# Aakash1312/Fluid-Simulation

Measured on AMD Instinct MI355X. Metric: simulated substeps/sec, higher is better.
Workload: dtype f64

## Files before the change

fluid-simulation_amd/csrc/common.h:

```cpp
#pragma once
#include <hip/hip_runtime.h>
#include <stdint.h>

namespace fl {

constexpr uint8_t F_SOLID = 1;
constexpr uint8_t F_FLUID = 2;
constexpr int F_CNT_SHIFT = 2;

struct Grid {
    int N;
    int lo;
    int hi;
    int nx, ny, nz;
    int ox, oy, oz;
    __host__ __device__ inline size_t idx(int ix, int iy, int iz) const
    {
        return ((size_t)ix * ny + (size_t)iy) * nz + (size_t)iz;
    }
    __host__ __device__ inline size_t cells() const { return (size_t)nx * ny * nz; }
    __host__ __device__ inline long sx() const { return (long)ny * nz; }
    __host__ __device__ inline int cx0() const { return lo + ox; }
    __host__ __device__ inline int cy0() const { return lo + oy; }
    __host__ __device__ inline int cz0() const { return lo + oz; }
// ... 115 lines not shown
    T r = 0;
    if (threadIdx.x == 0) {
#pragma unroll
        for (int i = 0; i < NW; ++i) r += sm[i];
    }
    return r;
}
template <int NW>
__device__ __forceinline__ double block_sum_array(const double* __restrict__ a, int n, double* sm)
{
    double v = 0;
    for (int i = threadIdx.x; i < n; i += NW * 64) v += a[i];
    v = wave_sum(v);
    const int lane = threadIdx.x & 63, w = threadIdx.x >> 6;
    __syncthreads();
    if (lane == 0) sm[w] = v;
    __syncthreads();
    if (threadIdx.x == 0) {
        double r = 0;
#pragma unroll
        for (int i = 0; i < NW; ++i) r += sm[i];
        sm[NW] = r;
    }
    __syncthreads();
    return sm[NW];
}

__device__ __forceinline__ int xcd_remap(int b, int nb)
{
    const int q = nb >> 3, r = nb & 7, xcd = b & 7;
    return (xcd < r ? xcd * (q + 1) : r * (q + 1) + (xcd - r) * q) + (b >> 3);
}

__device__ __forceinline__ void block_sum3(const double* __restrict__ a, int na, const double* __restrict__ b, int nb,
                                           const double* __restrict__ c, int nc, double* sm, double& ra, double& rb, double& rc)
{
    double va = 0, vb = 0, vc = 0;
    for (int i = threadIdx.x; i < na; i += 256) va += a[i];
    for (int i = threadIdx.x; i < nb; i += 256) vb += b[i];
    for (int i = threadIdx.x; i < nc; i += 256) vc += c[i];
    va = wave_sum(va); vb = wave_sum(vb); vc = wave_sum(vc);
    const int lane = threadIdx.x & 63, w = threadIdx.x >> 6;
    if (lane == 0) { sm[w] = va; sm[4 + w] = vb; sm[8 + w] = vc; }
    __syncthreads();
    ra = ((sm[0] + sm[1]) + sm[2]) + sm[3];
    rb = ((sm[4] + sm[5]) + sm[6]) + sm[7];
    rc = ((sm[8] + sm[9]) + sm[10]) + sm[11];
}

struct Particles {
    double *px, *py, *pz, *vx, *vy, *vz;
    uint32_t* pid;
    __host__ __device__ inline Particles shifted(long o) const
    {
        Particles q = *this;
        q.px += o; q.py += o; q.pz += o; q.vx += o; q.vy += o; q.vz += o; q.pid += o;
        return q;
    }
};
constexpr uint32_t PID_DEAD = 0xFFFFFFFFu;

void launch_bin_count(hipStream_t st, Grid g, long n, Particles p, int* key, int* slot, int* cell_count, int* part, StepState* ss);
void launch_bin_scatter(hipStream_t st, long n, const int* key, const int* slot, const int* cell_start, const uint32_t* pid, int* order,
                         uint32_t* spid);
void launch_bin_rank(hipStream_t st, long n_pos, long pos0, const int* key, const int* cell_start, const int* order, const uint32_t* spid,
                     int* order2);
void launch_reorder(hipStream_t st, long n, const int* order, Particles src, Particles dst, double* w = nullptr, long wstride = 0);
void launch_weights(hipStream_t st, long n, Particles p, double* w, long stride);
void launch_axpby_box(hipStream_t st, Grid g, Box box, double a, const double* x, double b, const double* y, double* out, const PcgState* gate = nullptr);
long p2g_max_items(Box box);
size_t p2g_part_doubles(Box box);
constexpr int P2G_PILED = 256;
void launch_p2g(hipStream_t st, Grid g, Box box, Particles p, const double* pw, long wstride, const int* cell_start, const uint8_t* flags,
                double* part, int* items, float* container, double* u, double* v, double* w, double* ub, double* vb, double* wb, int2* crowd_list = nullptr,
                Particles park = Particles{});
void launch_p2g_tiles(hipStream_t st, Grid g, Box box, Particles p, const double* pw, long wstride, const int* cell_start, const uint8_t* flags,
                      float* container, double* u, double* v, double* w, double* ub, double* vb, double* wb);
void launch_g2p_tiled(hipStream_t st, Grid g, Box pb, Particles p, const int* cell_start, const double* dcx, const double* dcy, const double* dcz,
                      const double* pcx, const double* pcy, const double* pcz, double blend, StepState* ss);
void launch_g2p(hipStream_t st, Grid g, long n, Particles p, const double* dcx, const double* dcy, const double* dcz, const double* pcx,
// ... 186 lines not shown
```

fluid-simulation_amd/csrc/kernels_mg.hip:

```cpp
#include "common.h"
#include <cstdlib>
#include <cstring>

namespace fl {

constexpr double MG_W1 = 0.5617, MG_W2 = 1.3895;

template <typename T>
__device__ __forceinline__ void mg_load_coef(T* sd, T* si, const MgCoef<T>& cf)
{
    if (threadIdx.x == 0) {
#pragma unroll
        for (int i = 0; i < 7; ++i) {
            sd[i] = cf.diag[i];
            si[i] = cf.inv[i];
        }
    }
    __syncthreads();
}

__device__ __forceinline__ bool mg_cell(const MLevel& m, long t, int& i, int& j, int& k)
{
    const unsigned n = (unsigned)m.dx * (unsigned)m.dy * (unsigned)m.dz;
    if (t >= (long)n) return false;
// ... 114 lines not shown
    z = r - y * RZ;
}
__device__ __forceinline__ bool in_level(const MLevel& m, int i, int j, int k)
{
    return (unsigned)i < (unsigned)m.dx && (unsigned)j < (unsigned)m.dy && (unsigned)k < (unsigned)m.dz;
}

__device__ __forceinline__ int clampi(int v, int hi) { return min(max(v, 0), hi); }

template <typename T, int TX, int TY, int TZ, bool RESTRICT>
struct DownTile {
    static constexpr int H = RESTRICT ? 3 : 2;
    static constexpr int AX = TX + 2 * H, AY = TY + 2 * H, AZ = TZ + 2 * H;
    static constexpr int BX = AX - 2, BY = AY - 2, BZ = AZ - 2;
    static constexpr int CX = BX - 2, CY = BY - 2, CZ = BZ - 2;
    static constexpr int nA = AX * AY * AZ, nB = BX * BY * BZ, nR = RESTRICT ? CX * CY * CZ : 4;
    static constexpr int oA = 0, oB = (oA + nA * (int)sizeof(T) + 15) / 16 * 16, oR = (oB + nB * (int)sizeof(T) + 15) / 16 * 16,
                         oC = (oR + nR * (int)sizeof(T) + 15) / 16 * 16, bytes = (oC + nA + 15) / 16 * 16;
};
template <typename T, int TX, int TY, int TZ>
struct UpTile {
    static constexpr int AX = TX + 4, AY = TY + 4, AZ = TZ + 4;
    static constexpr int BX = TX + 2, BY = TY + 2, BZ = TZ + 2;
    static constexpr int EX = TX / 2 + 4, EY = TY / 2 + 4, EZ = TZ / 2 + 4;
    static constexpr int nA = AX * AY * AZ, nB = BX * BY * BZ, nE = EX * EY * EZ;
    static constexpr int oA = 0, oB = (oA + nA * (int)sizeof(T) + 15) / 16 * 16, oE = (oB + nB * (int)sizeof(T) + 15) / 16 * 16,
                         oC = (oE + nE * (int)sizeof(T) + 15) / 16 * 16, bytes = (oC + nA + 15) / 16 * 16;
};

template <typename T, typename F, int TX, int TY, int TZ, bool RESTRICT, typename IO, int NG, typename RhsFn, typename CoreFn>
__device__ __forceinline__ void mg_down_body_fn(const MLevel& m, const uint8_t* __restrict__ cnt, T* __restrict__ u,
                                                T* __restrict__ r, const MLevel& mc, const uint8_t* __restrict__ cnt_c, T* __restrict__ fc,
                                                const MgCoef<T>* cf, T off, int tile, int gx, int gy, bool live, int col, char* lds, T* sd, T* si,
                                                int grp, RhsFn rhs, CoreFn core)
{
    typedef DownTile<T, TX, TY, TZ, RESTRICT> D;
    constexpr int H = D::H, AX = D::AX, AY = D::AY, AZ = D::AZ, BX = D::BX, BY = D::BY, BZ = D::BZ, CX = D::CX, CY = D::CY, CZ = D::CZ;
    constexpr int PA = (AX + NG - 1) / NG, PB = (BX + NG - 1) / NG;
    constexpr int NHC = NG * (256 / (CY * CZ)), XC = (CX + NHC - 1) / NHC;
    static_assert(AY * AZ <= 256 && NHC >= 1 && TX % 2 == 0 && TY % 2 == 0 && TZ % 2 == 0, "tile shape");
    T* sA = (T*)(lds + D::oA);
    T* sB = (T*)(lds + D::oB);
    T* sR = (T*)(lds + D::oR);
    uint8_t* sC = (uint8_t*)(lds + D::oC);
    const int tbx = tile % gx, tby = (tile / gx) % gy, tbz = tile / (gx * gy);
    const int i0 = tbz * TX, j0 = tby * TY, k0 = tbx * TZ;
    const T w1 = (T)MG_W1, w2 = (T)MG_W2;
    const long sx = m.sx;
    const int ya = col / AZ, za = col - ya * AZ;
    const bool actA = col < AY * AZ;
    const bool okA = actA && (unsigned)(j0 - H + ya) < (unsigned)m.dy && (unsigned)(k0 - H + za) < (unsigned)m.dz;
    const size_t qa = m.at(0, clampi(j0 - H + ya, m.dy - 1), clampi(k0 - H + za, m.dz - 1));
    const int xa0 = grp * PA;
    int ca[PA];
    T fa[PA];
#pragma unroll
    for (int p = 0; p < PA; ++p) {
        const int x = xa0 + p, i = i0 - H + x;
        const size_t q = qa + (size_t)((long)clampi(i, m.dx - 1) * sx);
        const int c = cnt[q];
        fa[p] = (T)rhs(q);
        ca[p] = (okA && x < AX && (unsigned)i < (unsigned)m.dx) ? c : 0;
    }
    const int yb = col / BZ, zb = col - yb * BZ;
    const bool actB = col < BY * BZ;
    const size_t qb = m.at(0, clampi(j0 - H + 1 + yb, m.dy - 1), clampi(k0 - H + 1 + zb, m.dz - 1));
    const int xb0 = grp * PB;
    T fb[PB];
#pragma unroll
    for (int p = 0; p < PB; ++p) fb[p] = (T)rhs(qb + (size_t)((long)clampi(i0 - H + 1 + xb0 + p, m.dx - 1) * sx));
    const int hc = grp * (256 / (CY * CZ)) + col / (CY * CZ), cc = col % (CY * CZ);
    const int yc = cc / CZ, zc = cc - yc * CZ;
    const bool actC = col / (CY * CZ) < 256 / (CY * CZ);
    const int xc0 = hc * XC;
    const size_t qc = m.at(0, clampi(j0 - H + 2 + yc, m.dy - 1), clampi(k0 - H + 2 + zc, m.dz - 1));
    T fr[XC];
#pragma unroll
    for (int x = 0; x < XC; ++x) fr[x] = (T)rhs(qc + (size_t)((long)clampi(i0 - H + 2 + xc0 + x, m.dx - 1) * sx));
    if (cf) mg_load_coef(sd, si, *cf);
    if (actA) {
#pragma unroll
        for (int p = 0; p < PA; ++p) {
            const int x = xa0 + p;
            if (x < AX) {
                sC[x * AY * AZ + col] = (uint8_t)ca[p];
                sA[x * AY * AZ + col] = w1 * si[ca[p]] * fa[p];
            }
        }
    }
    __syncthreads();
    if (actB && xb0 < BX) {
        const int a0 = (yb + 1) * AZ + zb + 1 + xb0 * AY * AZ;
        T cm = sA[a0], c0 = sA[a0 + AY * AZ];
        const bool in_yz = live && (unsigned)(yb - (H - 1)) < (unsigned)TY && (unsigned)(zb - (H - 1)) < (unsigned)TZ;
#pragma unroll
        for (int p = 0; p < PB; ++p) {
            const int x = xb0 + p;
            if (x < BX) {
                const int a = a0 + (p + 1) * AY * AZ;
                const T cp = sA[a + AY * AZ];
                const int n = sC[a];
                const T nb = cm + cp + sA[a - AZ] + sA[a + AZ] + sA[a - 1] + sA[a + 1];
                const T v = c0 + w2 * si[n] * (fb[p] - (sd[n] * c0 + off * nb));
                sB[(x * BY + yb) * BZ + zb] = v;
                if (n && in_yz && x >= H - 1 && x < H - 1 + TX) IO::st(u + qb + (size_t)((long)(i0 - H + 1 + x) * sx), v);
                cm = c0;
                c0 = cp;
            }
        }
    }
    __syncthreads();
    T rk[XC];
#pragma unroll
    for (int x = 0; x < XC; ++x) rk[x] = 0;
    if (actC && xc0 < CX) {
        const int b0 = ((xc0 + 1) * BY + yc + 1) * BZ + zc + 1;
        T cm = sB[b0 - BY * BZ], c0 = sB[b0];
#pragma unroll
        for (int x = 0; x < XC; ++x) {
            if (xc0 + x < CX) {
                const int b = b0 + x * BY * BZ;
                const T cp = sB[b + BY * BZ];
                const int n = sC[((xc0 + x + 2) * AY + yc + 2) * AZ + zc + 2];
// ... 31 lines not shown
            }
        }
    }
    if (RESTRICT) {
        __syncthreads();
        constexpr int QX = TX / 2, QY = TY / 2, QZ = TZ / 2;
        for (int t = grp * 256 + col; t < QX * QY * QZ; t += 256 * NG) {
            int X, Y, Z;
            region_cell<QY, QZ>(t, X, Y, Z);
            const int I = i0 / 2 + X, J = j0 / 2 + Y, K = k0 / 2 + Z;
            if (!live || !in_level(mc, I, J, K)) continue;
            const size_t C = mc.at(I, J, K);
            if (!cnt_c[C]) continue;
            auto w = [](int a) { return (a == 0 || a == 3) ? (T)0.25 : (T)0.75; };
            const T* p = sR + ((2 * X) * CY + 2 * Y) * CZ + 2 * Z;
            T acc = 0;
#pragma unroll
            for (int a = 0; a < 4; ++a) {
#pragma unroll
                for (int b = 0; b < 4; ++b) {
                    const T* q = p + (a * CY + b) * CZ;
                    acc += w(a) * w(b) * ((T)0.25 * (q[0] + q[3]) + (T)0.75 * (q[1] + q[2]));
                }
            }
            IO::st(fc + C, acc * (T)0.125);
        }
    }
}

template <typename T, typename F, int TX, int TY, int TZ, bool RESTRICT, typename IO, int NG = 1>
__device__ __forceinline__ void mg_down_body(const MLevel& m, const uint8_t* __restrict__ cnt, const F* __restrict__ f, T* __restrict__ u,
                                             T* __restrict__ r, const MLevel& mc, const uint8_t* __restrict__ cnt_c, T* __restrict__ fc,
                                             const MgCoef<T>* cf, T off, int tile, int gx, int gy, bool live, int col, char* lds, T* sd, T* si,
                                             int grp = 0)
{
    mg_down_body_fn<T, F, TX, TY, TZ, RESTRICT, IO, NG>(m, cnt, u, r, mc, cnt_c, fc, cf, off, tile, gx, gy, live, col, lds, sd, si, grp,
                                                        [&](size_t q) { return IO::ld(f + q); }, [](size_t) {});
}

template <typename T, typename F, int TX, int TY, int TZ, bool RESTRICT, int NG = 1>
__global__ __launch_bounds__(256 * NG) void k_mg_down(MLevel m, const uint8_t* __restrict__ cnt, const F* __restrict__ f, T* __restrict__ u,
                                                      T* __restrict__ r, MLevel mc, const uint8_t* __restrict__ cnt_c, T* __restrict__ fc,
                                                      MgCoef<T> cf, const PcgState* ps, int gx, int gy, const int* __restrict__ tlist)
{
    __shared__ __attribute__((aligned(16))) char lds[DownTile<T, TX, TY, TZ, RESTRICT>::bytes];
    __shared__ T sd[8], si[8];
    if (ps && ps->done) return;
    const int tile = tlist ? tlist[xcd_remap(blockIdx.x, gridDim.x)] : xcd_remap(blockIdx.x, gridDim.x);
    mg_down_body<T, F, TX, TY, TZ, RESTRICT, IoPlain, NG>(m, cnt, f, u, r, mc, cnt_c, fc, &cf, cf.off, tile, gx, gy, true, NG > 1 ? (int)(threadIdx.x & 255) : (int)threadIdx.x,
                                                          lds, sd, si, NG > 1 ? __builtin_amdgcn_readfirstlane(threadIdx.x >> 8) : 0);
}

template <typename T, typename F, typename O, int TX, int TY, int TZ, typename IO, int NG = 1>
__device__ __forceinline__ void mg_up_body(const MLevel& m, const uint8_t* __restrict__ cnt, const F* __restrict__ f, const T* __restrict__ u,
                                           O* __restrict__ out, const MLevel& mc, const T* __restrict__ ec, const MgCoef<T>* cf, T off,
                                           double* __restrict__ part_dot, int tile, int gx, int gy, T wc, const uint8_t* __restrict__ own, bool live,
                                           int col, char* lds, T* sd, T* si, double* red, int grp = 0, bool pconst = false)
{
    typedef UpTile<T, TX, TY, TZ> D;
    constexpr int AX = D::AX, AY = D::AY, AZ = D::AZ, BX = D::BX, BY = D::BY, BZ = D::BZ, EX = D::EX, EY = D::EY, EZ = D::EZ;
    constexpr int NE = (EX * EY * EZ + 256 * NG - 1) / (256 * NG);
    constexpr int PA = (AX + NG - 1) / NG, PB = (BX + NG - 1) / NG;
    constexpr int NHT = NG * (256 / (TY * TZ)), XT = (TX + NHT - 1) / NHT;
    static_assert(AY * AZ <= 256 && 256 % (TY * TZ) == 0 && TX % 2 == 0 && TY % 2 == 0 && TZ % 2 == 0, "tile shape");
    T* sA = (T*)(lds + D::oA);
    T* sB = (T*)(lds + D::oB);
    T* sE = (T*)(lds + D::oE);
    uint8_t* sC = (uint8_t*)(lds + D::oC);
    const int tbx = tile % gx, tby = (tile / gx) % gy, tbz = tile / (gx * gy);
    const int i0 = tbz * TX, j0 = tby * TY, k0 = tbx * TZ;
    const int I0 = i0 / 2 - 2, J0 = j0 / 2 - 2, K0 = k0 / 2 - 2;
    const long sx = m.sx;
    const int tid = grp * 256 + col;
    T ee[NE];
#pragma unroll
    for (int it = 0; it < NE; ++it) {
        int x, y, z;
        region_cell<EY, EZ>(tid + 256 * NG * it, x, y, z);
        const int I = I0 + x, J = J0 + y, K = K0 + z;
        const bool ok = I >= -1 && I <= mc.dx && J >= -1 && J <= mc.dy && K >= -1 && K <= mc.dz;
        const T v = IO::ld(ec + mc.at(min(max(I, -1), mc.dx), min(max(J, -1), mc.dy), min(max(K, -1), mc.dz)));
        ee[it] = ok ? v : (T)0;
    }
    const int ya = col / AZ, za = col - ya * AZ;
    const bool actA = col < AY * AZ;
    const bool okA = actA && (unsigned)(j0 - 2 + ya) < (unsigned)m.dy && (unsigned)(k0 - 2 + za) < (unsigned)m.dz;
    const size_t qa = m.at(0, clampi(j0 - 2 + ya, m.dy - 1), clampi(k0 - 2 + za, m.dz - 1));
    const int xa0 = grp * PA;
    int ca[PA];
    T ua[PA];
#pragma unroll
    for (int p = 0; p < PA; ++p) {
        const int x = xa0 + p, i = i0 - 2 + x;
        const size_t q = qa + (size_t)((long)clampi(i, m.dx - 1) * sx);
        const int c = cnt[q];
        ua[p] = IO::ld(u + q);
        ca[p] = (okA && (NG == 1 || x < AX) && (unsigned)i < (unsigned)m.dx) ? c : 0;
    }
    const int yb = col / BZ, zb = col - yb * BZ;
    const bool actB = col < BY * BZ;
    const size_t qb = m.at(0, clampi(j0 - 1 + yb, m.dy - 1), clampi(k0 - 1 + zb, m.dz - 1));
    const int xb0 = grp * PB;
    T fb[PB];
#pragma unroll
    for (int p = 0; p < PB; ++p) fb[p] = (T)IO::ld(f + qb + (size_t)((long)clampi(i0 - 1 + xb0 + p, m.dx - 1) * sx));
    const int hl = col / (TY * TZ), ct = col - hl * (TY * TZ);
    const int ht = NG == 1 ? hl : grp * (256 / (TY * TZ)) + hl;
    const int yt = ct / TZ, zt = ct - yt * TZ;
    const int xt0 = ht * XT;
    const size_t qt = m.at(0, clampi(j0 + yt, m.dy - 1), clampi(k0 + zt, m.dz - 1));
    F ft[XT];
#pragma unroll
    for (int x = 0; x < XT; ++x) ft[x] = IO::ld(f + qt + (size_t)((long)clampi(i0 + xt0 + x, m.dx - 1) * sx));
    if (cf) mg_load_coef(sd, si, *cf);
#pragma unroll
    for (int it = 0; it < NE; ++it) {
        const int t = tid + 256 * NG * it;
        if (t < EX * EY * EZ) sE[t] = ee[it];
    }
    __syncthreads();
    if (actA) {
        const int eb = ((ya >> 1) + 1) * EZ + (za >> 1) + 1;
        const int sy = (ya & 1) ? EZ : -EZ, sz = (za & 1) ? 1 : -1;
        const T a = (T)0.75, b = (T)0.25;
        T pl[EX];
#pragma unroll
        for (int I = 0; I < EX; ++I) {
            const T* p = sE + I * EY * EZ + eb;
            pl[I] = pconst ? p[0] : a * a * p[0] + a * b * (p[sy] + p[sz]) + b * b * p[sy + sz];
        }
#pragma unroll
        for (int p = 0; p < PA; ++p) {
            const int x = xa0 + p;
            if (NG == 1 || x < AX) {
                const int I = (x >> 1) + 1, In = (x & 1) ? I + 1 : I - 1;
                T pI = pl[0], pN = pl[0];
                if constexpr (NG == 1) {
                    pI = pl[(p >> 1) + 1], pN = pl[(p & 1) ? (p >> 1) + 2 : (p >> 1)];
                } else {
#pragma unroll
                    for (int e = 1; e < EX; ++e) { pI = e == I ? pl[e] : pI; pN = e == In ? pl[e] : pN; }
                }
                const T pe = pconst ? pI : a * pI + b * pN;
                sC[x * AY * AZ + col] = (uint8_t)ca[p];
                sA[x * AY * AZ + col] = ca[p] ? ua[p] + wc * pe : (T)0;
            }
        }
    }
    __syncthreads();
    if (actB && (NG == 1 || xb0 < BX)) {
        const int a0 = (yb + 1) * AZ + zb + 1 + xb0 * AY * AZ;
        T cm = sA[a0], c0 = sA[a0 + AY * AZ];
#pragma unroll
// ... 18 lines not shown
#pragma unroll
        for (int x = 0; x < XT; ++x) {
            if (NG == 1 || xt0 + x < TX) {
                const int b = b0 + x * BY * BZ;
                const T cp = sB[b + BY * BZ];
                const int n = sC[((xt0 + x + 2) * AY + yt + 2) * AZ + zt + 2];
                const T nb = cm + cp + sB[b - BZ] + sB[b + BZ] + sB[b - 1] + sB[b + 1];
                const T o = c0 + (T)MG_W1 * si[n] * ((T)ft[x] - (sd[n] * c0 + off * nb));
                if (n && live) {
                    const size_t qo = qt + (size_t)((long)(i0 + xt0 + x) * sx);
                    IO::st(out + qo, (O)o);
                    if (!own || (own[qo] && !(own[qo] & 0x80))) acc += (double)ft[x] * (double)o;
                }
                cm = c0;
                c0 = cp;
            }
        }
    }
    if (NG == 1 && part_dot) {
        acc = block_sum<double, 4>(acc, red);
        if (threadIdx.x == 0) part_dot[blockIdx.x] = acc;
    }
}

template <typename T, typename F, typename O, int TX, int TY, int TZ>
__global__ __launch_bounds__(256, 5) void k_mg_up(MLevel m, const uint8_t* __restrict__ cnt, const F* __restrict__ f, const T* __restrict__ u,
                                                                      O* __restrict__ out, MLevel mc, const T* __restrict__ ec, MgCoef<T> cf,
                                                                      double* __restrict__ part_dot, const PcgState* ps, int gx, int gy, T wc,
                                                                      const int* __restrict__ tlist, const uint8_t* __restrict__ own, int pconst)
{
    __shared__ __attribute__((aligned(16))) char lds[UpTile<T, TX, TY, TZ>::bytes];
    __shared__ T sd[8], si[8];
    __shared__ double red[4];
    if (ps && ps->done) return;
    const int tile = tlist ? tlist[xcd_remap(blockIdx.x, gridDim.x)] : xcd_remap(blockIdx.x, gridDim.x);
    mg_up_body<T, F, O, TX, TY, TZ, IoPlain, 1>(m, cnt, f, u, out, mc, ec, &cf, cf.off, part_dot, tile, gx, gy, wc, own, true, (int)threadIdx.x, lds, sd, si, red, 0,
                                                pconst != 0);
}

template <typename T>
__global__ __launch_bounds__(256) void k_mg_restrict(MLevel mf, const T* __restrict__ rf, MLevel mc, const uint8_t* __restrict__ cnt_c,
                                                     T* __restrict__ fc, const PcgState* ps)
{
    if (ps && ps->done) return;
    d_restrict<T>(mf, rf, mc, cnt_c, fc, (long)blockIdx.x * 256 + threadIdx.x);
}

constexpr int MG_TAIL_Q0 = 4;
template <typename T>
struct MgTail {
    int nl;
    MLevel mg[MG_TAIL_MAX];
    const uint8_t* cnt[MG_TAIL_MAX];
    const T* f0;
    T* u0;
    MLevel ml[MG_TAIL_MAX];
    int o_u[MG_TAIL_MAX], o_v[MG_TAIL_MAX], o_f[MG_TAIL_MAX], o_c[MG_TAIL_MAX];
    int lds_bytes;
    T off[MG_TAIL_MAX];
    int sweeps;
    double wc;
};

struct TailCell {
    int c;
    int n;
    int up;
    int down;
    int bits;
};
// ... 367 lines not shown
```

fluid-simulation_amd/csrc/kernels_pcg.hip:

```cpp
#include "common.h"
#include "stencil_vec.h"

namespace fl {

constexpr int TX = 4, TY = 8, TZ = 32;
constexpr int PY = TY + 2, PZ = TZ + 2;
constexpr int SQ_MAX_BLOCKS = 1024;
constexpr int XR_MAX_BLOCKS = 512;

LBox make_lbox(const Box& b)
{
    LBox L;
    L.x0 = b.x0; L.y0 = b.y0; L.z0 = b.z0;
    L.nx = b.nx(); L.ny = b.ny(); L.nz = b.nz();
    L.Lx = (L.nx + TX - 1) / TX * TX + 2;
    L.Ly = (L.ny + TY - 1) / TY * TY + 2;
    const int tiled = (L.nz + TZ - 1) / TZ * TZ + 1;
    const int need = LBOX_K0 + L.nz + 1 > tiled ? LBOX_K0 + L.nz + 1 : tiled;
    L.Lz = (need + 15) / 16 * 16;
    return L;
}
size_t lbox_max_cells(int N)
{
    Box b{0, 0, 0, N - 1, N - 1, N - 1};
// ... 73 lines not shown
    for (long t0 = (long)blockIdx.x * 256 + threadIdx.x; t0 < n; t0 += 4 * stride) {
        uint8_t c4[4];
#pragma unroll
        for (int q = 0; q < 4; ++q) { const long t = t0 + q * stride; c4[q] = cnt[t < n ? t : n - 1]; }
#pragma unroll
        for (int q = 0; q < 4; ++q) {
            const long t = t0 + q * stride;
            if (t >= n) break;
            const uint8_t c = c4[q];
            T rv = 0, xv = 0;
            if (c && !(c & 0x80)) {
                const int k = (int)(t % L.Lz), j = (int)((t / L.Lz) % L.Ly), i = (int)(t / ((long)L.Lz * L.Ly));
                const size_t gc = g.idx(L.x0 + i - 1, L.y0 + j - 1, L.z0 + k - LBOX_K0);
                const size_t gx = (size_t)g.sx(), gy = (size_t)g.nz;
                const T bv = (T)b[gc];
                auto G = [&](size_t q2) { return guess2 ? (T)(ca * guess[q2] + cb * guess2[q2]) : (T)guess[q2]; };
                const uint8_t n0 = cnt[t - sx], n1 = cnt[t + sx], n2 = cnt[t - sy], n3 = cnt[t + sy], n4 = cnt[t - 1], n5 = cnt[t + 1];
                const T g0 = G(gc - gx), g1 = G(gc + gx), g2 = G(gc - gy), g3 = G(gc + gy), g4 = G(gc - 1), g5 = G(gc + 1);
                xv = G(gc);
                const T nb = (n0 ? g0 : (T)0) + (n1 ? g1 : (T)0) + (n2 ? g2 : (T)0) + (n3 ? g3 : (T)0) + (n4 ? g4 : (T)0) + (n5 ? g5 : (T)0);
                rv = bv - (sdiag[c] * xv + cf.off * nb);
                abb += (double)bv * (double)bv;
                arr += (double)rv * (double)rv;
            }
            x[t] = xv;
            r[t] = rv;
        }
    }
    abb = block_sum<double, 4>(abb, red);
    arr = block_sum<double, 4>(arr, red);
    if (threadIdx.x == 0) { part_bb[blockIdx.x] = abb; part_rr0[blockIdx.x] = arr; }
}

template <typename T>
__device__ __forceinline__ bool pcg_head(const double* __restrict__ part_rr, const double* __restrict__ part_rz_new,
                                         const double* __restrict__ part_rz_old, int n_prev, int n_rz, PcgState* ps, int first, double tol,
                                         double* red, T& beta)
{
    const int tid = threadIdx.x;
    beta = 0;
    if (first) {
        double bb, rr0, d2;
        block_sum3(part_rr, n_prev, part_rz_old, first == 2 ? n_prev : 0, part_rr, 0, red, bb, rr0, d2);
        if (first != 2) rr0 = bb;
        const bool go = bb > 0 && !(rr0 < tol * tol * bb);
        if (blockIdx.x == 0 && tid == 0) {
            ps->bb = bb;
            ps->thr = tol * tol * bb;
            ps->rr = rr0;
            if (!go) ps->done = 1;
        }
        return go;
    }
    double rr, rzn, rzo;
    block_sum3(part_rr, n_prev, part_rz_new, n_rz, part_rz_old, n_rz, red, rr, rzn, rzo);
    if (rr < ps->thr) {
        if (blockIdx.x == 0 && tid == 0) { ps->rr = rr; ps->done = 1; }
        return false;
    }
    beta = (T)(rzn / rzo);
    if (blockIdx.x == 0 && tid == 0) { ps->rr = rr; ps->iters += 1; }
    return true;
}

template <typename T, bool DIST, bool AZ = false, typename ZT = T>
__global__ __launch_bounds__(256) void k_pcg_sq_l(LBox L, const uint8_t* __restrict__ cnt, const ZT* __restrict__ r,
                                                  const T* __restrict__ s_in, T* __restrict__ s_out, T* __restrict__ q, Coef<T> cf,
                                                  const double* __restrict__ part_rr, const double* __restrict__ part_rz_new,
                                                  const double* __restrict__ part_rz_old, double* __restrict__ part_pq, int n_prev,
                                                  PcgState* ps, int first, double tol, int n_rz, int zmode, int sparse,
                                                  const int* __restrict__ tlist, int nlist)
{
    __shared__ T sT[TX * PY * PZ];
    __shared__ double red[16];
    __shared__ int s_done;
    __shared__ T sdiag[8], sinv[8];
    const int tid = threadIdx.x;
    load_coef(sdiag, sinv, cf);
    if (tid == 0) s_done = ps->done;

    const int nty = (L.ny + TY - 1) / TY, ntz = (L.nz + TZ - 1) / TZ;
    const int ntiles = ((L.nx + TX - 1) / TX) * nty * ntz;
    const long sx = (long)L.Ly * L.Lz;
    const int ly = tid >> 5, kz = tid & 31;

    int lidx = xcd_remap(blockIdx.x, gridDim.x);
    int tile = tlist ? (lidx < nlist ? tlist[lidx] : ntiles) : lidx;
    auto entry = [&](int li) { return tlist ? (li < nlist ? tlist[li < nlist ? li : 0] : ntiles) : li; };
    int nxt = entry(lidx + (int)gridDim.x);
    uint8_t fc[TX + 2], fy = 0, fz = 0;
    ZT rv[TX + 2], ry = 0, rz = 0;
    T sv[TX + 2], sy = 0, sz = 0;
    long c0 = 0;
    auto issue = [&](int tl, bool counts, bool values) {
        const int tz = tl % ntz, ty = (tl / ntz) % nty, tx = tl / (ntz * nty);
        const int i0 = 1 + tx * TX, j0 = 1 + ty * TY, k0 = LBOX_K0 + tz * TZ;
        c0 = ((long)(i0 - 1) * L.Ly + (j0 + ly)) * L.Lz + k0 + kz;
#pragma unroll
        for (int m = 0; m < TX + 2; ++m) {
            if (counts) fc[m] = cnt[c0 + m * sx];
            if (values) {
                rv[m] = r[c0 + m * sx];
                sv[m] = first ? (T)0 : s_in[c0 + m * sx];
            }
        }
        {
            const int pl = tid >> 6, side = (tid >> 5) & 1;
            const long cy = ((long)(i0 + pl) * L.Ly + (side ? j0 + TY : j0 - 1)) * L.Lz + k0 + kz;
            if (counts) fy = cnt[cy];
            if (values) { ry = r[cy]; sy = first ? (T)0 : s_in[cy]; }
        }
        if (tid < 64) {
            const int lx = tid >> 4, l2 = (tid >> 1) & 7, side = tid & 1;
            const long cz = ((long)(i0 + lx) * L.Ly + (j0 + l2)) * L.Lz + (side ? k0 + TZ : k0 - 1);
            if (counts) fz = cnt[cz];
            if (values) { rz = r[cz]; sz = first ? (T)0 : s_in[cz]; }
        }
    };
    if (!sparse && tile < ntiles) issue(tile, true, true);

    T beta = 0;
    __syncthreads();
    if (s_done) return;
    if (!AZ && !pcg_head<T>(part_rr, part_rz_new, part_rz_old, n_prev, n_rz, ps, first, tol, red, beta)) return;

    double acc = 0;
    while (tile < ntiles) {
        if (sparse) {
            issue(tile, true, false);
            int any = 0;
#pragma unroll
            for (int m = 1; m <= TX; ++m) any |= fc[m];
            if (!__syncthreads_or(any)) {
                tile = nxt;
                lidx += gridDim.x;
                nxt = entry(lidx + (int)gridDim.x);
                continue;
            }
            issue(tile, false, true);
        }
        T val[TX + 2];
#pragma unroll
        for (int m = 0; m < TX + 2; ++m) val[m] = fc[m] ? (zmode ? (T)rv[m] : (T)rv[m] * sinv[DIST ? fc[m] & 7 : fc[m]]) + beta * sv[m] : (T)0;
#pragma unroll
        for (int lx = 0; lx < TX; ++lx) sT[(lx * PY + ly + 1) * PZ + kz + 1] = val[lx + 1];
        {
            const int pl = tid >> 6, side = (tid >> 5) & 1;
            sT[(pl * PY + (side ? TY + 1 : 0)) * PZ + kz + 1] = fy ? (zmode ? (T)ry : (T)ry * sinv[DIST ? fy & 7 : fy]) + beta * sy : (T)0;
        }
        if (tid < 64) {
            const int lx = tid >> 4, l2 = (tid >> 1) & 7, side = tid & 1;
            sT[(lx * PY + l2 + 1) * PZ + (side ? TZ + 1 : 0)] = fz ? (zmode ? (T)rz : (T)rz * sinv[DIST ? fz & 7 : fz]) + beta * sz : (T)0;
        }
        __syncthreads();
        const long cc = c0;
        uint8_t fcc[TX];
        T nbv[TX], cen[TX];
// ... 131 lines not shown
        }
        ((V2*)s)[i] = sv; ((V2*)q)[i] = qv; ((V2*)x)[i] = xv; ((V2*)r)[i] = rv;
    }
    arr = block_sum<double, 4>(arr, red);
    if (threadIdx.x == 0) part_rr[blockIdx.x] = arr;
}

__global__ __launch_bounds__(256) void k_pcg_poll_stage(const double* __restrict__ part_rr, int n, const PcgState* ps, double* __restrict__ out)
{
    __shared__ double red[16];
    double ra, rb, rc;
    block_sum3(part_rr, n, part_rr, 0, part_rr, 0, red, ra, rb, rc);
    if (threadIdx.x == 0) {
        out[0] = ra;
        out[1] = ps->done ? 1.0 : 0.0;
    }
}
__global__ void k_pcg_poll_test(const double* __restrict__ g, PcgState* ps)
{
    if (g[1] > 0) ps->done = 1;
    else if (g[0] < ps->thr) { ps->rr = g[0]; ps->done = 1; }
}

template <typename T, bool SPARSE>
__global__ __launch_bounds__(256) void k_pcg_xr_l(long n2, const uint8_t* __restrict__ cnt, T* __restrict__ x, T* __restrict__ r,
                                                  const T* __restrict__ s, const T* __restrict__ q, Coef<T> cf,
                                                  const double* __restrict__ part_rz_cur, int n_xr, const double* __restrict__ part_pq,
                                                  int n_sq, double* __restrict__ part_rr, double* __restrict__ part_rz_next, PcgState* ps,
                                                  int dist)
{
    __shared__ double red[16];
    __shared__ int s_done;
    __shared__ T sdiag[8], sinv[8];
    load_coef(sdiag, sinv, cf);
    if (threadIdx.x == 0) s_done = ps->done;
    typedef Vec2<T> V2;
    const V2* x2 = (const V2*)x;
    const V2* r2 = (const V2*)r;
    const V2* s2 = (const V2*)s;
    const V2* q2 = (const V2*)q;
    const uint16_t* c2 = (const uint16_t*)cnt;
    const int vb = xcd_remap(blockIdx.x, gridDim.x);
    const long per = (n2 + gridDim.x - 1) / gridDim.x;
    const long e0 = (long)vb * per, e1 = e0 + per < n2 ? e0 + per : n2;
    constexpr int U = 4;
    V2 xv[U], rv[U], sv[U], qv[U];
    uint16_t cv[U];
    long i = e0 + threadIdx.x;
    auto issue = [&](long base) {
#pragma unroll
        for (int u = 0; u < U; ++u) {
            const long e = base + u * 256, ec = e < n2 ? e : n2 - 1;
            cv[u] = c2[ec];
            if (!SPARSE) { xv[u] = x2[ec]; rv[u] = r2[ec]; sv[u] = s2[ec]; qv[u] = q2[ec]; }
        }
        if (SPARSE) {
#pragma unroll
            for (int u = 0; u < U; ++u) {
                const long e = base + u * 256;
                if (e >= e1) cv[u] = 0;
                if (cv[u]) { xv[u] = x2[e]; rv[u] = r2[e]; sv[u] = s2[e]; qv[u] = q2[e]; }
            }
        }
    };
    issue(i);
    __syncthreads();
    if (s_done) return;
    double rz, pq, d3;
    block_sum3(part_rz_cur, n_xr, part_pq, n_sq, part_pq, 0, red, rz, pq, d3);
    if (!(pq > 0) || !(rz == rz)) {
        if (blockIdx.x == 0 && threadIdx.x == 0) { ps->breakdown = 1; ps->done = 1; }
        return;
    }
    const T alpha = (T)(rz / pq);
    double arr = 0, arz = 0;
    for (; i < e1; i += U * 256) {
        V2 xo[U], ro[U];
        uint16_t cw[U];
#pragma unroll
        for (int u = 0; u < U; ++u) {
            cw[u] = i + u * 256 < e1 ? cv[u] : (uint16_t)0;
            xo[u] = xv[u]; ro[u] = rv[u];
            if (cw[u]) {
                int ca = cw[u] & 0xff, cb = cw[u] >> 8;
                if (dist) { ca = (ca & 0x80) ? 0 : ca; cb = (cb & 0x80) ? 0 : cb; }
                if (ca) {
                    xo[u].a = xo[u].a + alpha * sv[u].a;
                    ro[u].a = ro[u].a - alpha * qv[u].a;
                    const T z = ro[u].a * sinv[ca];
                    arr += (double)ro[u].a * (double)ro[u].a;
                    arz += (double)ro[u].a * (double)z;
                }
                if (cb) {
                    xo[u].b = xo[u].b + alpha * sv[u].b;
                    ro[u].b = ro[u].b - alpha * qv[u].b;
                    const T z = ro[u].b * sinv[cb];
                    arr += (double)ro[u].b * (double)ro[u].b;
                    arz += (double)ro[u].b * (double)z;
                }
            }
        }
        const long ib = i;
        if (!SPARSE || i + U * 256 < e1) issue(i + U * 256);
#pragma unroll
        for (int u = 0; u < U; ++u)
            if (cw[u]) {
                ((V2*)x)[ib + u * 256] = xo[u];
                ((V2*)r)[ib + u * 256] = ro[u];
            }
    }
    arr = block_sum<double, 4>(arr, red);
    arz = block_sum<double, 4>(arz, red);
    if (threadIdx.x == 0) { part_rr[blockIdx.x] = arr; part_rz_next[blockIdx.x] = arz; }
}


template <typename T>
__global__ __launch_bounds__(256) void k_pcg_xr_t(LBox L, const uint8_t* __restrict__ cnt, T* __restrict__ x, T* __restrict__ r,
                                                  const T* __restrict__ s, const T* __restrict__ q, Coef<T> cf,
                                                  const double* __restrict__ part_rz_cur, int n_xr, const double* __restrict__ part_pq,
                                                  int n_sq, double* __restrict__ part_rr, double* __restrict__ part_rz_next, PcgState* ps,
                                                  const int* __restrict__ tlist, int nlist)
{
    __shared__ double red[16];
    __shared__ int s_done;
    __shared__ T sdiag[8], sinv[8];
    load_coef(sdiag, sinv, cf);
    if (threadIdx.x == 0) s_done = ps->done;
    const int nty = (L.ny + TY - 1) / TY, ntz = (L.nz + TZ - 1) / TZ;
    const long sx = (long)L.Ly * L.Lz;
    const int ly = threadIdx.x >> 5, kz = threadIdx.x & 31;
    uint8_t cv[TX];
    T xv[TX], rv[TX], sv[TX], qv[TX];
    long c0 = 0;
    auto issue = [&](int tl) {
        const int tz = tl % ntz, ty = (tl / ntz) % nty, tx = tl / (ntz * nty);
        c0 = ((long)(1 + tx * TX) * L.Ly + (1 + ty * TY + ly)) * L.Lz + LBOX_K0 + tz * TZ + kz;
#pragma unroll
        for (int m = 0; m < TX; ++m) {
            const long c = c0 + m * sx;
            cv[m] = cnt[c];
            xv[m] = x[c]; rv[m] = r[c]; sv[m] = s[c]; qv[m] = q[c];
        }
    };
    int lidx = xcd_remap(blockIdx.x, gridDim.x);
    if (lidx < nlist) issue(tlist[lidx]);
    __syncthreads();
    if (s_done) return;
    double rz, pq, d3;
    block_sum3(part_rz_cur, n_xr, part_pq, n_sq, part_pq, 0, red, rz, pq, d3);
    if (!(pq > 0) || !(rz == rz)) {
        if (blockIdx.x == 0 && threadIdx.x == 0) { ps->breakdown = 1; ps->done = 1; }
        return;
    }
    const T alpha = (T)(rz / pq);
    double arr = 0, arz = 0;
    while (lidx < nlist) {
        const long cc = c0;
        uint8_t cw[TX];
        T xo[TX], ro[TX];
#pragma unroll
        for (int m = 0; m < TX; ++m) {
            cw[m] = cv[m];
            xo[m] = xv[m] + alpha * sv[m];
            ro[m] = rv[m] - alpha * qv[m];
        }
        lidx += gridDim.x;
        if (lidx < nlist) issue(tlist[lidx]);
#pragma unroll
        for (int m = 0; m < TX; ++m) {
            if (cw[m]) {
                const T z = ro[m] * sinv[cw[m]];
                arr += (double)ro[m] * (double)ro[m];
                arz += (double)ro[m] * (double)z;
                x[cc + m * sx] = xo[m];
                r[cc + m * sx] = ro[m];
            }
        }
    }
    arr = block_sum<double, 4>(arr, red);
    arz = block_sum<double, 4>(arz, red);
    if (threadIdx.x == 0) { part_rr[blockIdx.x] = arr; part_rz_next[blockIdx.x] = arz; }
}

template <typename T>
__global__ __launch_bounds__(256) void k_pcg_xr_rows(LBox L, const uint8_t* __restrict__ cnt, T* __restrict__ x, T* __restrict__ r,
                                                     const T* __restrict__ s, const T* __restrict__ q, Coef<T> cf,
                                                     const double* __restrict__ part_rz_cur, int n_xr, const double* __restrict__ part_pq,
                                                     int n_sq, double* __restrict__ part_rr, double* __restrict__ part_rz_next, PcgState* ps,
                                                     const int* __restrict__ rlist, int nrows)
{
    __shared__ double red[16];
    __shared__ int s_done;
    __shared__ T sdiag[8], sinv[8];
    load_coef(sdiag, sinv, cf);
    if (threadIdx.x == 0) s_done = ps->done;
    const int ntz = (L.nz + 31) / 32;
    const int sub = threadIdx.x >> 5, kz = threadIdx.x & 31;
    constexpr int U = 2;
    long c[U];
    uint8_t cv[U];
    T xv[U], rv[U], sv[U], qv[U];
    int rown[U];
    const int stride = gridDim.x * 8;
    int ri = xcd_remap(blockIdx.x, gridDim.x) * 8 + sub;
    auto row_at = [&](int rr) { return rlist[rr < nrows ? rr : nrows - 1]; };
    auto cell_row = [&](int row) {
        const int tz = row % ntz, iy = (row / ntz) % L.ny, ix = row / (ntz * L.ny);
        return ((long)(1 + ix) * L.Ly + (1 + iy)) * L.Lz + LBOX_K0 + tz * 32 + kz;
    };
    auto issue = [&](int u, int row) {
        c[u] = cell_row(row);
        cv[u] = cnt[c[u]];
        xv[u] = x[c[u]]; rv[u] = r[c[u]]; sv[u] = s[c[u]]; qv[u] = q[c[u]];
    };
#pragma unroll
    for (int u = 0; u < U; ++u) rown[u] = row_at(ri + u * stride);
#pragma unroll
    for (int u = 0; u < U; ++u) {
        issue(u, rown[u]);
        rown[u] = row_at(ri + (U + u) * stride);
    }
    __syncthreads();
    if (s_done) return;
    double rz, pq, d3;
    block_sum3(part_rz_cur, n_xr, part_pq, n_sq, part_pq, 0, red, rz, pq, d3);
    if (!(pq > 0) || !(rz == rz)) {
        if (blockIdx.x == 0 && threadIdx.x == 0) { ps->breakdown = 1; ps->done = 1; }
        return;
    }
    const T alpha = (T)(rz / pq);
    double arr = 0, arz = 0;
    for (; ri < nrows; ri += U * stride) {
#pragma unroll
        for (int u = 0; u < U; ++u) {
            const long cc = c[u];
            const uint8_t cw = ri + u * stride < nrows ? cv[u] : (uint8_t)0;
            const T xo = xv[u] + alpha * sv[u], ro = rv[u] - alpha * qv[u];
            issue(u, rown[u]);
            rown[u] = row_at(ri + (2 * U + u) * stride);
            if (cw) {
                const T z = ro * sinv[cw];
                arr += (double)ro * (double)ro;
                arz += (double)ro * (double)z;
                x[cc] = xo;
                r[cc] = ro;
            }
        }
    }
    arr = block_sum<double, 4>(arr, red);
    arz = block_sum<double, 4>(arz, red);
    if (threadIdx.x == 0) { part_rr[blockIdx.x] = arr; part_rz_next[blockIdx.x] = arz; }
}
__global__ __launch_bounds__(256) void k_row_flags(LBox L, const uint8_t* __restrict__ cnt, int nrows_all, int* __restrict__ flags)
{
    const int row = blockIdx.x * 8 + (threadIdx.x >> 5), kz = threadIdx.x & 31;
    const int ntz = (L.nz + 31) / 32;
    int any = 0;
    if (row < nrows_all) {
// ... 345 lines not shown
```

Baseline: 155.9.

## Prefetch reduction partials and done flag before coefficient load in PCG/MG kernels

Splits block_sum3 into a load phase and a sum phase so that the partial-sum reads and the PcgState done/thr flags are issued at kernel entry, overlapping their latency with coefficient loading and the first tile fetches. MG smoother kernels now read the done flag with a relaxed atomic load and defer the early exit until after the tile loads, instead of blocking on the flag up front. The intent is to hide the serial global-load latency at the head of each small CG/MG kernel. The cost is extra registers for the prefetched values and, when the solver is already done, wasted tile loads.

```diff
diff --git a/fluid-simulation_amd/csrc/common.h b/fluid-simulation_amd/csrc/common.h
--- a/fluid-simulation_amd/csrc/common.h
+++ b/fluid-simulation_amd/csrc/common.h
@@ -171,13 +171,48 @@
     return (xcd < r ? xcd * (q + 1) : r * (q + 1) + (xcd - r) * q) + (b >> 3);
 }
 
-__device__ __forceinline__ void block_sum3(const double* __restrict__ a, int na, const double* __restrict__ b, int nb,
-                                           const double* __restrict__ c, int nc, double* sm, double& ra, double& rb, double& rc)
-{
-    double va = 0, vb = 0, vc = 0;
-    for (int i = threadIdx.x; i < na; i += 256) va += a[i];
-    for (int i = threadIdx.x; i < nb; i += 256) vb += b[i];
-    for (int i = threadIdx.x; i < nc; i += 256) vc += c[i];
+template <typename X>
+__device__ __forceinline__ X vload(const X* p)
+{
+    return __hip_atomic_load(p, __ATOMIC_RELAXED, __HIP_MEMORY_SCOPE_AGENT);
+}
+
+constexpr int SUM3_PRE = 4;
+struct Sum3Loads {
+    double a[SUM3_PRE], b[SUM3_PRE], c[SUM3_PRE];
+};
+__device__ __forceinline__ void sum3_load1(const double* __restrict__ a, int n, double* v)
+{
+    const int last = n > 0 ? n - 1 : 0;
+#pragma unroll
+    for (int k = 0; k < SUM3_PRE; ++k) {
+        const int i = (int)threadIdx.x + 256 * k;
+        v[k] = a[i < last ? i : last];
+    }
+}
+template <bool LATE_C = false>
+__device__ __forceinline__ void block_sum3_load(const double* __restrict__ a, int na, const double* __restrict__ b, int nb,
+                                                const double* __restrict__ c, int nc, Sum3Loads& v)
+{
+    sum3_load1(a, na, v.a);
+    sum3_load1(nb > 0 ? b : a, nb, v.b);
+    if (!LATE_C) sum3_load1(nc > 0 ? c : a, nc, v.c);
+}
+__device__ __forceinline__ double sum3_thread(const double* __restrict__ a, int n, const double* v)
+{
+    double s = 0;
+#pragma unroll
+    for (int k = 0; k < SUM3_PRE; ++k)
+        if ((int)threadIdx.x + 256 * k < n) s += v[k];
+    for (int i = (int)threadIdx.x + 256 * SUM3_PRE; i < n; i += 256) s += a[i];
+    return s;
+}
+template <bool LATE_C = false>
+__device__ __forceinline__ void block_sum3_sum(Sum3Loads& v, const double* __restrict__ a, int na, const double* __restrict__ b, int nb,
+                                               const double* __restrict__ c, int nc, double* sm, double& ra, double& rb, double& rc)
+{
+    if (LATE_C) sum3_load1(nc > 0 ? c : a, nc, v.c);
+    double va = sum3_thread(a, na, v.a), vb = sum3_thread(b, nb, v.b), vc = sum3_thread(c, nc, v.c);
     va = wave_sum(va); vb = wave_sum(vb); vc = wave_sum(vc);
     const int lane = threadIdx.x & 63, w = threadIdx.x >> 6;
     if (lane == 0) { sm[w] = va; sm[4 + w] = vb; sm[8 + w] = vc; }
@@ -185,6 +220,13 @@
     ra = ((sm[0] + sm[1]) + sm[2]) + sm[3];
     rb = ((sm[4] + sm[5]) + sm[6]) + sm[7];
     rc = ((sm[8] + sm[9]) + sm[10]) + sm[11];
+}
+__device__ __forceinline__ void block_sum3(const double* __restrict__ a, int na, const double* __restrict__ b, int nb,
+                                           const double* __restrict__ c, int nc, double* sm, double& ra, double& rb, double& rc)
+{
+    Sum3Loads v;
+    block_sum3_load(a, na, b, nb, c, nc, v);
+    block_sum3_sum(v, a, na, b, nb, c, nc, sm, ra, rb, rc);
 }
 
 struct Particles {
diff --git a/fluid-simulation_amd/csrc/kernels_mg.hip b/fluid-simulation_amd/csrc/kernels_mg.hip
--- a/fluid-simulation_amd/csrc/kernels_mg.hip
+++ b/fluid-simulation_amd/csrc/kernels_mg.hip
@@ -170,7 +170,7 @@
 __device__ __forceinline__ void mg_down_body_fn(const MLevel& m, const uint8_t* __restrict__ cnt, T* __restrict__ u,
                                                 T* __restrict__ r, const MLevel& mc, const uint8_t* __restrict__ cnt_c, T* __restrict__ fc,
                                                 const MgCoef<T>* cf, T off, int tile, int gx, int gy, bool live, int col, char* lds, T* sd, T* si,
-                                                int grp, RhsFn rhs, CoreFn core)
+                                                int grp, int dn, RhsFn rhs, CoreFn core)
 {
     typedef DownTile<T, TX, TY, TZ, RESTRICT> D;
     constexpr int H = D::H, AX = D::AX, AY = D::AY, AZ = D::AZ, BX = D::BX, BY = D::BY, BZ = D::BZ, CX = D::CX, CY = D::CY, CZ = D::CZ;
@@ -227,6 +227,7 @@
         }
     }
     __syncthreads();
+    if (dn) return;
     if (actB && xb0 < BX) {
         const int a0 = (yb + 1) * AZ + zb + 1 + xb0 * AY * AZ;
         T cm = sA[a0], c0 = sA[a0 + AY * AZ];
@@ -324,9 +325,9 @@
 __device__ __forceinline__ void mg_down_body(const MLevel& m, const uint8_t* __restrict__ cnt, const F* __restrict__ f, T* __restrict__ u,
                                              T* __restrict__ r, const MLevel& mc, const uint8_t* __restrict__ cnt_c, T* __restrict__ fc,
                                              const MgCoef<T>* cf, T off, int tile, int gx, int gy, bool live, int col, char* lds, T* sd, T* si,
-                                             int grp = 0)
-{
-    mg_down_body_fn<T, F, TX, TY, TZ, RESTRICT, IO, NG>(m, cnt, u, r, mc, cnt_c, fc, cf, off, tile, gx, gy, live, col, lds, sd, si, grp,
+                                             int grp, int dn)
+{
+    mg_down_body_fn<T, F, TX, TY, TZ, RESTRICT, IO, NG>(m, cnt, u, r, mc, cnt_c, fc, cf, off, tile, gx, gy, live, col, lds, sd, si, grp, dn,
                                                         [&](size_t q) { return IO::ld(f + q); }, [](size_t) {});
 }
 
@@ -337,17 +338,22 @@
 {
     __shared__ __attribute__((aligned(16))) char lds[DownTile<T, TX, TY, TZ, RESTRICT>::bytes];
     __shared__ T sd[8], si[8];
-    if (ps && ps->done) return;
+    int dn = 0;
+    if constexpr (RESTRICT) {
+        if (ps && ps->done) return;
+    } else {
+        dn = vload(&ps->done);
+    }
     const int tile = tlist ? tlist[xcd_remap(blockIdx.x, gridDim.x)] : xcd_remap(blockIdx.x, gridDim.x);
     mg_down_body<T, F, TX, TY, TZ, RESTRICT, IoPlain, NG>(m, cnt, f, u, r, mc, cnt_c, fc, &cf, cf.off, tile, gx, gy, true, NG > 1 ? (int)(threadIdx.x & 255) : (int)threadIdx.x,
-                                                          lds, sd, si, NG > 1 ? __builtin_amdgcn_readfirstlane(threadIdx.x >> 8) : 0);
+                                                          lds, sd, si, NG > 1 ? __builtin_amdgcn_readfirstlane(threadIdx.x >> 8) : 0, dn);
 }
 
 template <typename T, typename F, typename O, int TX, int TY, int TZ, typename IO, int NG = 1>
 __device__ __forceinline__ void mg_up_body(const MLevel& m, const uint8_t* __restrict__ cnt, const F* __restrict__ f, const T* __restrict__ u,
                                            O* __restrict__ out, const MLevel& mc, const T* __restrict__ ec, const MgCoef<T>* cf, T off,
                                            double* __restrict__ part_dot, int tile, int gx, int gy, T wc, const uint8_t* __restrict__ own, bool live,
-                                           int col, char* lds, T* sd, T* si, double* red, int grp = 0, bool pconst = false)
+                                           int col, char* lds, T* sd, T* si, double* red, int grp, bool pconst, int dn)
 {
     typedef UpTile<T, TX, TY, TZ> D;
     constexpr int AX = D::AX, AY = D::AY, AZ = D::AZ, BX = D::BX, BY = D::BY, BZ = D::BZ, EX = D::EX, EY = D::EY, EZ = D::EZ;
@@ -411,6 +417,7 @@
         if (t < EX * EY * EZ) sE[t] = ee[it];
     }
     __syncthreads();
+    if (dn) return;
     if (actA) {
         const int eb = ((ya >> 1) + 1) * EZ + (za >> 1) + 1;
         const int sy = (ya & 1) ? EZ : -EZ, sz = (za & 1) ? 1 : -1;
@@ -495,10 +502,10 @@
     __shared__ __attribute__((aligned(16))) char lds[UpTile<T, TX, TY, TZ>::bytes];
     __shared__ T sd[8], si[8];
     __shared__ double red[4];
-    if (ps && ps->done) return;
+    const int dn = vload(&ps->done);
     const int tile = tlist ? tlist[xcd_remap(blockIdx.x, gridDim.x)] : xcd_remap(blockIdx.x, gridDim.x);
     mg_up_body<T, F, O, TX, TY, TZ, IoPlain, 1>(m, cnt, f, u, out, mc, ec, &cf, cf.off, part_dot, tile, gx, gy, wc, own, true, (int)threadIdx.x, lds, sd, si, red, 0,
-                                                pconst != 0);
+                                                pconst != 0, dn);
 }
 
 template <typename T>
diff --git a/fluid-simulation_amd/csrc/kernels_pcg.hip b/fluid-simulation_amd/csrc/kernels_pcg.hip
--- a/fluid-simulation_amd/csrc/kernels_pcg.hip
+++ b/fluid-simulation_amd/csrc/kernels_pcg.hip
@@ -129,8 +129,20 @@
     if (threadIdx.x == 0) { part_bb[blockIdx.x] = abb; part_rr0[blockIdx.x] = arr; }
 }
 
-template <typename T>
-__device__ __forceinline__ bool pcg_head(const double* __restrict__ part_rr, const double* __restrict__ part_rz_new,
+struct HeadLoads {
+    Sum3Loads p;
+    double thr;
+};
+template <bool LATE_C>
+__device__ __forceinline__ void pcg_head_load(const double* __restrict__ part_rr, const double* __restrict__ part_rz_new,
+                                              const double* __restrict__ part_rz_old, int n_prev, int n_rz, const PcgState* ps, int first, HeadLoads& h)
+{
+    h.thr = vload(&ps->thr);
+    const double* pb = first ? part_rz_old : part_rz_new;
+    block_sum3_load<LATE_C>(part_rr, n_prev, pb, first ? (first == 2 ? n_prev : 0) : n_rz, part_rz_old, first ? 0 : n_rz, h.p);
+}
+template <typename T, bool LATE_C>
+__device__ __forceinline__ bool pcg_head(HeadLoads& h, const double* __restrict__ part_rr, const double* __restrict__ part_rz_new,
                                          const double* __restrict__ part_rz_old, int n_prev, int n_rz, PcgState* ps, int first, double tol,
                                          double* red, T& beta)
 {
@@ -138,7 +150,7 @@
     beta = 0;
     if (first) {
         double bb, rr0, d2;
-        block_sum3(part_rr, n_prev, part_rz_old, first == 2 ? n_prev : 0, part_rr, 0, red, bb, rr0, d2);
+        block_sum3_sum<LATE_C>(h.p, part_rr, n_prev, part_rz_old, first == 2 ? n_prev : 0, part_rr, 0, red, bb, rr0, d2);
         if (first != 2) rr0 = bb;
         const bool go = bb > 0 && !(rr0 < tol * tol * bb);
         if (blockIdx.x == 0 && tid == 0) {
@@ -150,8 +162,8 @@
         return go;
     }
     double rr, rzn, rzo;
-    block_sum3(part_rr, n_prev, part_rz_new, n_rz, part_rz_old, n_rz, red, rr, rzn, rzo);
-    if (rr < ps->thr) {
+    block_sum3_sum<LATE_C>(h.p, part_rr, n_prev, part_rz_new, n_rz, part_rz_old, n_rz, red, rr, rzn, rzo);
+    if (rr < h.thr) {
         if (blockIdx.x == 0 && tid == 0) { ps->rr = rr; ps->done = 1; }
         return false;
     }
@@ -173,8 +185,11 @@
     __shared__ int s_done;
     __shared__ T sdiag[8], sinv[8];
     const int tid = threadIdx.x;
+    const int dn = vload(&ps->done);
+    HeadLoads hl;
+    constexpr bool LATE_C = sizeof(T) == 4;
+    if constexpr (!AZ) pcg_head_load<LATE_C>(part_rr, part_rz_new, part_rz_old, n_prev, n_rz, ps, first, hl);
     load_coef(sdiag, sinv, cf);
-    if (tid == 0) s_done = ps->done;
 
     const int nty = (L.ny + TY - 1) / TY, ntz = (L.nz + TZ - 1) / TZ;
     const int ntiles = ((L.nx + TX - 1) / TX) * nty * ntz;
@@ -215,11 +230,14 @@
         }
     };
     if (!sparse && tile < ntiles) issue(tile, true, true);
+    if (tid == 0) s_done = dn;
 
     T beta = 0;
     __syncthreads();
     if (s_done) return;
-    if (!AZ && !pcg_head<T>(part_rr, part_rz_new, part_rz_old, n_prev, n_rz, ps, first, tol, red, beta)) return;
+    if constexpr (!AZ) {
+        if (!pcg_head<T, LATE_C>(hl, part_rr, part_rz_new, part_rz_old, n_prev, n_rz, ps, first, tol, red, beta)) return;
+    }
 
     double acc = 0;
     while (tile < ntiles) {
@@ -417,8 +435,10 @@
     __shared__ double red[16];
     __shared__ int s_done;
     __shared__ T sdiag[8], sinv[8];
+    const int dn = vload(&ps->done);
+    Sum3Loads pl;
+    block_sum3_load(part_rz_cur, n_xr, part_pq, n_sq, part_pq, 0, pl);
     load_coef(sdiag, sinv, cf);
-    if (threadIdx.x == 0) s_done = ps->done;
     typedef Vec2<T> V2;
     const V2* x2 = (const V2*)x;
     const V2* r2 = (const V2*)r;
@@ -449,10 +469,11 @@
         }
     };
     issue(i);
+    if (threadIdx.x == 0) s_done = dn;
     __syncthreads();
     if (s_done) return;
     double rz, pq, d3;
-    block_sum3(part_rz_cur, n_xr, part_pq, n_sq, part_pq, 0, red, rz, pq, d3);
+    block_sum3_sum(pl, part_rz_cur, n_xr, part_pq, n_sq, part_pq, 0, red, rz, pq, d3);
     if (!(pq > 0) || !(rz == rz)) {
         if (blockIdx.x == 0 && threadIdx.x == 0) { ps->breakdown = 1; ps->done = 1; }
         return;
@@ -510,8 +531,10 @@
     __shared__ double red[16];
     __shared__ int s_done;
     __shared__ T sdiag[8], sinv[8];
+    const int dn = vload(&ps->done);
+    Sum3Loads pl;
+    block_sum3_load(part_rz_cur, n_xr, part_pq, n_sq, part_pq, 0, pl);
     load_coef(sdiag, sinv, cf);
-    if (threadIdx.x == 0) s_done = ps->done;
     const int nty = (L.ny + TY - 1) / TY, ntz = (L.nz + TZ - 1) / TZ;
     const long sx = (long)L.Ly * L.Lz;
     const int ly = threadIdx.x >> 5, kz = threadIdx.x & 31;
@@ -530,10 +553,11 @@
     };
     int lidx = xcd_remap(blockIdx.x, gridDim.x);
     if (lidx < nlist) issue(tlist[lidx]);
+    if (threadIdx.x == 0) s_done = dn;
     __syncthreads();
     if (s_done) return;
     double rz, pq, d3;
-    block_sum3(part_rz_cur, n_xr, part_pq, n_sq, part_pq, 0, red, rz, pq, d3);
+    block_sum3_sum(pl, part_rz_cur, n_xr, part_pq, n_sq, part_pq, 0, red, rz, pq, d3);
     if (!(pq > 0) || !(rz == rz)) {
         if (blockIdx.x == 0 && threadIdx.x == 0) { ps->breakdown = 1; ps->done = 1; }
         return;
@@ -578,8 +602,10 @@
     __shared__ double red[16];
     __shared__ int s_done;
     __shared__ T sdiag[8], sinv[8];
+    const int dn = vload(&ps->done);
+    Sum3Loads pl;
+    block_sum3_load(part_rz_cur, n_xr, part_pq, n_sq, part_pq, 0, pl);
     load_coef(sdiag, sinv, cf);
-    if (threadIdx.x == 0) s_done = ps->done;
     const int ntz = (L.nz + 31) / 32;
     const int sub = threadIdx.x >> 5, kz = threadIdx.x & 31;
     constexpr int U = 2;
@@ -606,10 +632,11 @@
         issue(u, rown[u]);
         rown[u] = row_at(ri + (U + u) * stride);
     }
+    if (threadIdx.x == 0) s_done = dn;
     __syncthreads();
     if (s_done) return;
     double rz, pq, d3;
-    block_sum3(part_rz_cur, n_xr, part_pq, n_sq, part_pq, 0, red, rz, pq, d3);
+    block_sum3_sum(pl, part_rz_cur, n_xr, part_pq, n_sq, part_pq, 0, red, rz, pq, d3);
     if (!(pq > 0) || !(rz == rz)) {
         if (blockIdx.x == 0 && threadIdx.x == 0) { ps->breakdown = 1; ps->done = 1; }
         return;
```

Result: faster. 158.6 (median of 6 runs) (+1.7%).
